# taldatech/soft-intro-vae-pytorch

Hardware: AMD Instinct MI355X
Metric: training images/sec (whole node) at 256x256 bs128 (higher is better)
Workload: dtype f32; 1 GPU; soft_intro_vae celeb256 256x256 zdim=512 channels=[64, 128, 256, 512, 512, 512], full E-step + D-step iteration; global_batch=128, per_gpu_batch=128, parallelism=dp1, decoder_forward_reuse=True, hip_graph=False, batchnorm=local

## Files before the change

### soft-intro-vae-pytorch_amd/csrc/bn_fused.hip

```cpp
#include "bn_fused_common.h"
#include <stdlib.h>

namespace {

struct BnFusedArgs {
  const float* dy;
  const float* y;
  const float* x;
  const unsigned char* mask;
  const float* mean;
  const float* invstd;
  const float* gamma;
  const float* beta;
  float* dx;
  float* dz;
  float* dgamma;
  float* dbeta;
  double* part;
  double* sums;
  unsigned* bar;
  double count;
  float slope;
  int C, H, W, Bs, nseg;
  int l2_qpp, l2_qw;
  int spc, cpg, ngroups, nx;
  int nsub;
  int local;
  int dzmode;
  int pf;
  unsigned spin_limit;
#ifdef BF_TIMING
  unsigned long long* ts;
#endif
};
#ifdef BF_TIMING
#define BF_STAMP(K) \
  if (t == 0 && a.ts) a.ts[((size_t)blockIdx.x * a.ngroups + grp) * 8 + (K)] = __builtin_amdgcn_s_memrealtime();
#else
#define BF_STAMP(K)
#endif

__device__ __forceinline__ void bf_sign_nibble(float4& g, unsigned nib, float slope) {
  g.x = (nib & 1u) ? g.x : g.x * slope;
  g.y = (nib & 2u) ? g.y : g.y * slope;
  g.z = (nib & 4u) ? g.z : g.z * slope;
  g.w = (nib & 8u) ? g.w : g.w * slope;
}
__device__ __forceinline__ void bf_sign_val(float4& g, const float4 v, float slope) {
  g.x = v.x > 0.f ? g.x : g.x * slope;
  g.y = v.y > 0.f ? g.y : g.y * slope;
  g.z = v.z > 0.f ? g.z : g.z * slope;
  g.w = v.w > 0.f ? g.w : g.w * slope;
}
__device__ __forceinline__ void bf_store4(__amdgpu_buffer_rsrc_t r, const float4 v, unsigned voff, unsigned soff) {
  typedef unsigned int u32x4_t __attribute__((ext_vector_type(4)));
  f32x4 f;
  f[0] = v.x;
  f[1] = v.y;
  f[2] = v.z;
  f[3] = v.w;
  __builtin_amdgcn_raw_buffer_store_b128(__builtin_bit_cast(u32x4_t, f), r, (int)voff, (int)soff, 0);
}
#define BF_KEEP(V) asm volatile("" ::"v"((V).x), "v"((V).y), "v"((V).z), "v"((V).w));

template <int ACT, bool POOL, int NQ>
__global__ void __launch_bounds__(256, 2) bn_bwd_fused_kernel(BnFusedArgs a) {
  __shared__ double red[8];
  extern __shared__ __attribute__((aligned(16))) float4 bf_pfx[];
  const int t = threadIdx.x;
  const int wave64 = __builtin_amdgcn_readfirstlane(t >> 6) * 64;
  const bool pf = NQ <= 8 && a.pf != 0;
  constexpr int PFQ = NQ < 6 ? NQ : 6;
  const bool local = a.local != 0;
  const int nb_sub = local ? (int)gridDim.x : (int)gridDim.x / a.nsub;
  const int sub = (!local && (int)blockIdx.x >= nb_sub) ? 1 : 0;
  const int bid = (int)blockIdx.x - sub * nb_sub;
  unsigned* bar = a.bar + sub * BF_BAR_UINTS;
  unsigned* chcnt = a.bar + 2 * BF_BAR_UINTS;
  const int xcd = bid % a.nx;
  const unsigned bpx = (unsigned)(nb_sub / a.nx);
  __shared__ int bar_failed;
  unsigned target = 0, nbar = 0;
  if (t == 0 && !local) target = bf_load_u32(bar + (9 + xcd) * 32);
  const int C = a.C, W = a.W, HW = a.H * a.W;
  const int VC = a.nseg * C;
  const int nq = a.Bs << a.l2_qpp;
  const unsigned qpp_m = (1u << a.l2_qpp) - 1u, qw_m = (1u << a.l2_qw) - 1u;
  const int ci = local ? 0 : bid / a.spc, slab = local ? 0 : bid - ci * a.spc;
  const float slope = a.slope;
  const unsigned img_pitch = (unsigned)C * (unsigned)HW * 4u;
  const unsigned row_b = (unsigned)W * 4u;
  const unsigned long long win = ((unsigned long long)(a.Bs - 1) * C + 1ull) * HW * 4ull;

  float4 g0[NQ], g1[NQ], x0[NQ], x1[NQ];
#pragma unroll
  for (int j = 0; j < NQ; ++j) g0[j] = g1[j] = x0[j] = x1[j] = make_float4(0.f, 0.f, 0.f, 0.f);
  const unsigned qbase = (unsigned)(slab * (256 * NQ) + t);
  auto quad_off = [&](unsigned q) -> unsigned {
    const unsigned b = q >> a.l2_qpp, r = q & qpp_m, h2 = r >> a.l2_qw, w4 = r & qw_m;
    const unsigned off = b * img_pitch + (2u * h2 * (unsigned)W + 4u * w4) * 4u;
    return q < (unsigned)nq ? off : BF_OOB;
  };
  auto half_off = [&](unsigned q) -> unsigned {
    const unsigned b = q >> a.l2_qpp, r = q & qpp_m, h2 = r >> a.l2_qw, w4 = r & qw_m;
    const unsigned off = b * (img_pitch >> 2) + (h2 * (unsigned)(W >> 1) + 2u * w4) * 4u;
    return q < (unsigned)nq ? off : BF_OOB;
  };
  auto request_x = [&](int vcn) {
    const int segn = vcn / C, cn = vcn - segn * C;
    const __amdgpu_buffer_rsrc_t rxn = make_rsrc(a.x + ((size_t)segn * a.Bs * C + cn) * (size_t)HW, win);
#pragma unroll
    for (int j = 0; j < PFQ; ++j) {
      const unsigned vo = quad_off(qbase + j * 256);
      __builtin_amdgcn_raw_ptr_buffer_load_lds(rxn, (float __attribute__((address_space(3)))*)(bf_pfx + (2 * j) * 256 + wave64),
                                               16, (int)vo, 0, 0, 0);
      __builtin_amdgcn_raw_ptr_buffer_load_lds(rxn, (float __attribute__((address_space(3)))*)(bf_pfx + (2 * j + 1) * 256 + wave64),
                                               16, (int)vo, (int)row_b, 0, 0);
    }
  };
  if (pf && !local && ci < a.cpg && sub * a.cpg + ci < VC && sub < a.ngroups) request_x(sub * a.cpg + ci);
  for (int grp = sub; grp < (local ? 1 : a.ngroups); grp += a.nsub) {
    const int vc = local ? bid : grp * a.cpg + ci;
    const bool active = local ? true : (ci < a.cpg && vc < VC);
    double t1 = 0.0, t2 = 0.0;
    float m = 0.f, is = 0.f, gs = 0.f;
    int c = 0;
    size_t base = 0;
    BF_STAMP(0)
    if (active) {
      const int seg = vc / C;
      c = vc - seg * C;
      m = a.mean[vc];
      is = a.invstd[vc];
      gs = a.gamma[c] * is;
      const float bt = ACT == 2 ? a.beta[c] : 0.f;
      base = ((size_t)seg * a.Bs * C + c) * (size_t)HW;
      const __amdgpu_buffer_rsrc_t rx = make_rsrc(a.x + base, win);
      const __amdgpu_buffer_rsrc_t rdy = POOL ? make_rsrc(a.dy + (base >> 2), win >> 2) : make_rsrc(a.dy + base, win);
      unsigned nib[ACT == 3 ? NQ : 1];
#pragma unroll
      for (int j = 0; j < NQ; ++j) {
        const unsigned vo = quad_off(qbase + j * 256);
        BF_KEEP(x0[j]) BF_KEEP(x1[j]) BF_KEEP(g0[j]) BF_KEEP(g1[j])
        if (!pf || j >= PFQ) {
          x0[j] = buf_load_f32x4(rx, vo, 0);
          x1[j] = buf_load_f32x4(rx, vo, row_b);
        }
        if (POOL) {
          const float2 d = buf_load_f32x2(rdy, half_off(qbase + j * 256), 0);
          g0[j] = make_float4(0.25f * d.x, 0.25f * d.x, 0.25f * d.y, 0.25f * d.y);
          g1[j] = g0[j];
        } else {
          g0[j] = buf_load_f32x4(rdy, vo, 0);
          g1[j] = buf_load_f32x4(rdy, vo, row_b);
        }
        if (ACT == 3) {
          const __amdgpu_buffer_rsrc_t rm = make_rsrc(a.mask + (base >> 3), win >> 5);
          const unsigned mo = vo == BF_OOB ? BF_OOB : (vo >> 5);
          const unsigned b0_ = (unsigned)__builtin_amdgcn_raw_buffer_load_b8(rm, (int)mo, 0, 0);
          const unsigned b1_ = (unsigned)__builtin_amdgcn_raw_buffer_load_b8(rm, (int)mo, (int)(W >> 3), 0);
          nib[j] = b0_ | (b1_ << 8);
        }
        if (ACT == 1) {
          const __amdgpu_buffer_rsrc_t ry = make_rsrc(a.y + base, win);
          bf_sign_val(g0[j], buf_load_f32x4(ry, vo, 0), slope);
          bf_sign_val(g1[j], buf_load_f32x4(ry, vo, row_b), slope);
        }
      }
      if (pf) {
#pragma unroll
        for (int j = 0; j < PFQ; ++j) {
          x0[j] = bf_pfx[(2 * j) * 256 + t];
          x1[j] = bf_pfx[(2 * j + 1) * 256 + t];
        }
      }
      double s1 = 0.0, s2 = 0.0;
#ifdef BF_TIMING
      asm volatile("s_waitcnt vmcnt(0)" ::: "memory");
#endif
      BF_STAMP(1)
#pragma unroll
      for (int j = 0; j < NQ; ++j) {
        if (ACT == 3) {
          const unsigned sh = (quad_off(qbase + j * 256) >> 4) & 1u ? 4u : 0u;
          bf_sign_nibble(g0[j], (nib[j] >> sh) & 0xfu, slope);
          bf_sign_nibble(g1[j], (nib[j] >> (8u + sh)) & 0xfu, slope);
        }
        if (ACT == 2) {
          float4 v = make_float4((x0[j].x - m) * gs + bt, (x0[j].y - m) * gs + bt, (x0[j].z - m) * gs + bt,
                                 (x0[j].w - m) * gs + bt);
          bf_sign_val(g0[j], v, slope);
          v = make_float4((x1[j].x - m) * gs + bt, (x1[j].y - m) * gs + bt, (x1[j].z - m) * gs + bt,
                          (x1[j].w - m) * gs + bt);
          bf_sign_val(g1[j], v, slope);
        }
        x0[j] = make_float4((x0[j].x - m) * is, (x0[j].y - m) * is, (x0[j].z - m) * is, (x0[j].w - m) * is);
        x1[j] = make_float4((x1[j].x - m) * is, (x1[j].y - m) * is, (x1[j].z - m) * is, (x1[j].w - m) * is);
        const float q1 = ((g0[j].x + g0[j].y) + (g0[j].z + g0[j].w)) + ((g1[j].x + g1[j].y) + (g1[j].z + g1[j].w));
        const float q2 = ((g0[j].x * x0[j].x + g0[j].y * x0[j].y) + (g0[j].z * x0[j].z + g0[j].w * x0[j].w)) +
                         ((g1[j].x * x1[j].x + g1[j].y * x1[j].y) + (g1[j].z * x1[j].z + g1[j].w * x1[j].w));
        s1 += (double)q1;
        s2 += (double)q2;
      }
      block_sum2<256>(s1, s2, red);
      if (local) {
        t1 = s1;
        t2 = s2;
      } else if (t == 0) {
        __hip_atomic_store(a.part + ((size_t)vc * a.spc + slab) * 2 + 0, s1, __ATOMIC_RELAXED, __HIP_MEMORY_SCOPE_AGENT);
        __hip_atomic_store(a.part + ((size_t)vc * a.spc + slab) * 2 + 1, s2, __ATOMIC_RELAXED, __HIP_MEMORY_SCOPE_AGENT);
      }
    }
    BF_STAMP(2)
    if (!local) {
      if (t == 0) {
        ++target;
        bf_grid_arrive(bar, xcd, a.nx, bpx, nbar++);
      }
      BF_STAMP(3)
      if (pf) {
        const int vcn = (grp + a.nsub) * a.cpg + ci;
        if (grp + a.nsub < a.ngroups && ci < a.cpg && vcn < VC) request_x(vcn);
      }
      if (t == 0) bar_failed = bf_grid_wait(bar, a.bar + BF_POISON_WORD, xcd, target, a.spin_limit) ? 0 : 1;
      BF_STAMP(4)
      __syncthreads();
      if (bar_failed) return;
      if (!active) continue;
      for (int s = t; s < a.spc; s += 512) {
        const int sb = s + 256 < a.spc ? s + 256 : s;
        const double p1 = bf_load_f64(a.part + ((size_t)vc * a.spc + s) * 2 + 0);
        const double p2 = bf_load_f64(a.part + ((size_t)vc * a.spc + s) * 2 + 1);
        const double q1 = bf_load_f64(a.part + ((size_t)vc * a.spc + sb) * 2 + 0);
        const double q2 = bf_load_f64(a.part + ((size_t)vc * a.spc + sb) * 2 + 1);
        t1 += p1;
        t2 += p2;
        if (s + 256 < a.spc) {
          t1 += q1;
          t2 += q2;
        }
      }
      block_sum2<256>(t1, t2, red);
    }
    const float c1 = (float)(t1 / a.count), c2 = (float)(t2 / a.count);
    BF_STAMP(5)
    if (slab == 0 && t == 0 && (a.dgamma != nullptr || a.dbeta != nullptr)) {
      if (a.nseg == 1) {
        if (a.dbeta) a.dbeta[c] = (float)t1;
        if (a.dgamma) a.dgamma[c] = (float)t2;
      } else {
        __hip_atomic_store(a.sums + (size_t)vc * 2 + 0, t1, __ATOMIC_RELAXED, __HIP_MEMORY_SCOPE_AGENT);
        __hip_atomic_store(a.sums + (size_t)vc * 2 + 1, t2, __ATOMIC_RELAXED, __HIP_MEMORY_SCOPE_AGENT);
        asm volatile("s_waitcnt vmcnt(0)" ::: "memory");
        const unsigned done = __hip_atomic_fetch_add(chcnt + c, 1u, __ATOMIC_RELAXED, __HIP_MEMORY_SCOPE_AGENT);
        if (done == (unsigned)a.nseg - 1u) {
          double u1 = 0.0, u2 = 0.0;
          for (int g = 0; g < a.nseg; ++g) {
            u1 += bf_load_f64(a.sums + (size_t)(g * C + c) * 2 + 0);
            u2 += bf_load_f64(a.sums + (size_t)(g * C + c) * 2 + 1);
          }
          if (a.dbeta) a.dbeta[c] = (float)u1;
          if (a.dgamma) a.dgamma[c] = (float)u2;
          __hip_atomic_store(chcnt + c, 0u, __ATOMIC_RELAXED, __HIP_MEMORY_SCOPE_AGENT);
        }
      }
    }
    const __amdgpu_buffer_rsrc_t rdx = make_rsrc(a.dx + base, win);
    const __amdgpu_buffer_rsrc_t rdz = a.dzmode == 2 ? make_rsrc(a.dz + (base >> 2), win >> 2)
                                                     : make_rsrc(a.dzmode == 1 ? a.dz + base : a.dx + base, win);
#pragma unroll
    for (int j = 0; j < NQ; ++j) {
      const unsigned vo = quad_off(qbase + j * 256);
      x0[j].x = gs * (g0[j].x - c1 - x0[j].x * c2);
      x0[j].y = gs * (g0[j].y - c1 - x0[j].y * c2);
      x0[j].z = gs * (g0[j].z - c1 - x0[j].z * c2);
      x0[j].w = gs * (g0[j].w - c1 - x0[j].w * c2);
      x1[j].x = gs * (g1[j].x - c1 - x1[j].x * c2);
      x1[j].y = gs * (g1[j].y - c1 - x1[j].y * c2);
      x1[j].z = gs * (g1[j].z - c1 - x1[j].z * c2);
      x1[j].w = gs * (g1[j].w - c1 - x1[j].w * c2);
      if (vo == BF_OOB) continue;
      bf_store4(rdx, x0[j], vo, 0);
      bf_store4(rdx, x1[j], vo, row_b);
      if (a.dzmode == 1) {
        bf_store4(rdz, g0[j], vo, 0);
        bf_store4(rdz, g1[j], vo, row_b);
      } else if (a.dzmode == 2) {
        const float sa = (g0[j].x + g0[j].y) + (g1[j].x + g1[j].y);
        const float sb = (g0[j].z + g0[j].w) + (g1[j].z + g1[j].w);
        buf_store_f32x2(rdz, sa, sb, half_off(qbase + j * 256), 0);
      }
    }
    BF_STAMP(6)
#ifdef BF_TIMING
    asm volatile("s_waitcnt vmcnt(0)" ::: "memory");
    BF_STAMP(7)
#endif
  }
  if (t == 0 && bid == 0 && nbar != 0u) bf_grid_reset(bar, a.nx);
  asm volatile("s_waitcnt vmcnt(0)" ::: "memory");
#pragma unroll
  for (int j = 0; j < NQ; ++j) { BF_KEEP(x0[j]) BF_KEEP(x1[j]) BF_KEEP(g0[j]) BF_KEEP(g1[j]) }
}

struct BfPlan {
  int nq_per_thread;
  int spc, cpg, ngroups, nb_sub, nsub;
  int local;
};

static bool bf_occupancy_ok() {
  static int ok = -1;
  if (ok < 0) {
    int ndev = 0, n = 0;
    if (hipGetDeviceCount(&ndev) != hipSuccess || ndev <= 0) {
      (void)hipGetLastError();
      ok = 1;
    } else {
      hipError_t e = hipSuccess;
      int n8 = 0;
      if (e == hipSuccess) e = hipOccupancyMaxActiveBlocksPerMultiprocessor(&n8, bn_bwd_fused_kernel<3, false, 8>, 256, 48 * 1024);
      if (e == hipSuccess) e = hipOccupancyMaxActiveBlocksPerMultiprocessor(&n, bn_bwd_fused_kernel<3, false, 10>, 256, 0);
      if (e == hipSuccess && n8 < n) n = n8;
      ok = (e != hipSuccess || n >= 2) ? 1 : 0;
      if (e != hipSuccess) (void)hipGetLastError();
    }
  }
  return ok == 1;
}

static bool bf_plan(int Bs, int VC, int HW, int max_nq, BfPlan* out) {
  const long long nq = (long long)Bs * HW / 8;
  out->local = 0;
  for (int NQ : {4, 8, 10}) {
    if (NQ > max_nq || nq > 256LL * NQ) continue;
    out->nq_per_thread = NQ;
    out->spc = 1;
    out->cpg = 1;
    out->ngroups = VC;
    out->nb_sub = VC;
    out->nsub = 1;
    out->local = 1;
    return true;
  }
  if (!bf_persistent_allowed() || !bf_occupancy_ok()) return false;
  for (int nsub = 2; nsub >= 1; --nsub) {
    const int nb_sub = sivae_num_cus() * (nsub == 2 ? 1 : 2);
    double best = 0.0;
    bool found = false;
    static int force_nq = -1;
    if (force_nq < 0) {
      const char* e = getenv("SIVAE_BN_FUSED_NQ");
      force_nq = e ? atoi(e) : 0;
    }
    for (int NQ : {10, 8, 4}) {
      if (NQ > max_nq) continue;
      if (force_nq > 0 && NQ != force_nq && NQ <= max_nq && force_nq <= max_nq) continue;
      const long long slabq = 256LL * NQ;
      const long long spc = (nq + slabq - 1) / slabq;
      if (spc > nb_sub) continue;
      const int cpg = (int)(nb_sub / spc);
      const int ngroups = (VC + cpg - 1) / cpg;
      const double cost = (double)((ngroups + nsub - 1) / nsub) * (8.0 + 2.5 * NQ);
      if (!found || cost < best) {
        best = cost;
        found = true;
        out->nq_per_thread = NQ;
        out->spc = (int)spc;
        out->cpg = cpg;
        out->ngroups = ngroups;
        out->nb_sub = nb_sub;
        out->nsub = nsub;
      }
    }
    if (found) return true;
  }
  return false;
}

static inline bool is_pow2(int v) { return v > 0 && (v & (v - 1)) == 0; }

#ifdef BF_TIMING
static unsigned long long* bf_timing_buffer = nullptr;
#endif

}

#ifdef BF_TIMING
extern "C" void sivae_debug_bf_timing(unsigned long long* buf) { bf_timing_buffer = buf; }
extern "C" int sivae_debug_bf_plan(int B, int C, int H, int W, int seg_images, int max_nq, int* out6) {
  BfPlan p;
  if (!bf_plan(seg_images, (B / seg_images) * C, H * W, max_nq, &p)) return -1;
  out6[0] = p.nq_per_thread; out6[1] = p.spc; out6[2] = p.cpg; out6[3] = p.ngroups; out6[4] = p.nb_sub; out6[5] = p.nsub;
  return 0;
}
#endif

extern "C" int sivae_bn_bwd_fused_supported(int B, int C, int H, int W, int seg_images) {
  if (B <= 0 || C <= 0 || C > BF_CH_COUNTERS || !is_pow2(H) || !is_pow2(W) || H < 2 || W < 4) return 0;
  if (seg_images <= 0 || B % seg_images != 0) return 0;
  if ((long long)B * C * H * W >= 0xffffffffLL) return 0;
  if ((long long)seg_images * C * H * W * 4 >= 0xfffffe00LL) return 0;
  BfPlan p;
  return bf_plan(seg_images, (B / seg_images) * C, H * W, 8, &p) ? 1 : 0;
}

extern "C" int sivae_bn_bwd_fused_poison_word() { return BF_POISON_WORD; }

extern "C" size_t sivae_bn_bwd_fused_workspace_bytes(int B, int C, int H, int W, int seg_images) {
  if (!sivae_bn_bwd_fused_supported(B, C, H, W, seg_images)) return 0;
  const int VC = (B / seg_images) * C;
  BfPlan p;
  size_t worst = 0;
  for (int mq : {10, 8, 4})
    if (bf_plan(seg_images, VC, H * W, mq, &p) && (size_t)p.spc > worst) worst = (size_t)p.spc;
  return ((size_t)VC * worst * 2 + (size_t)VC * 2) * sizeof(double);
}

extern "C" int sivae_bn_bwd_fused_state_uints() { return 2 * BF_BAR_UINTS + BF_CH_COUNTERS; }

extern "C" int sivae_bn_bwd_fused(const float* dy, const float* y, const unsigned char* mask, const float* x,
                                  const float* mean, const float* invstd, const float* gamma, const float* beta,
                                  int act_mode, float slope, float* dx, float* dz_out, float* dgamma, float* dbeta, int B,
                                  int C, int H, int W, int dy_pooled, int dz_sum, int seg_images, unsigned int* state,
                                  void* workspace, size_t workspace_bytes, hipStream_t stream) {
  if (!dy || !x || !mean || !invstd || !gamma || !dx || !state) return SIVAE_ERR_NULL;
  if (act_mode < 0 || act_mode > 3) return SIVAE_ERR_MODE;
  if (act_mode == 1 && !y) return SIVAE_ERR_NULL;
  if (act_mode == 2 && !beta) return SIVAE_ERR_NULL;
  if (act_mode == 3 && !mask) return SIVAE_ERR_NULL;
  if (act_mode == 3 && (W & 7)) return SIVAE_ERR_SHAPE;
  if (dy_pooled && dz_sum) return SIVAE_ERR_MODE;
  if (dz_sum && !dz_out) return SIVAE_ERR_NULL;
  if (!sivae_bn_bwd_fused_supported(B, C, H, W, seg_images)) return SIVAE_ERR_SHAPE;
  if (((uintptr_t)dy & 15u) || ((uintptr_t)x & 15u) || ((uintptr_t)dx & 15u) || (dz_out && ((uintptr_t)dz_out & 15u)) ||
      (y && ((uintptr_t)y & 15u)))
    return SIVAE_ERR_SHAPE;
  const int nseg = B / seg_images, VC = nseg * C;
  BfPlan p;
  if (!bf_plan(seg_images, VC, H * W, act_mode == 1 ? 8 : 10, &p)) return SIVAE_ERR_SHAPE;
  const size_t need = ((size_t)VC * p.spc * 2 + (size_t)VC * 2) * sizeof(double);
  if (!workspace || workspace_bytes < need) return SIVAE_ERR_WORKSPACE;
  BnFusedArgs a;
  a.dy = dy;
  a.y = y;
  a.x = x;
  a.mask = mask;
  a.mean = mean;
  a.invstd = invstd;
  a.gamma = gamma;
  a.beta = beta;
  a.dx = dx;
  a.dz = dz_out;
  a.dgamma = dgamma;
  a.dbeta = dbeta;
  a.part = (double*)workspace;
  a.sums = a.part + (size_t)VC * p.spc * 2;
  a.bar = state;
  a.count = (double)seg_images * H * W;
  a.slope = slope;
  a.C = C;
  a.H = H;
  a.W = W;
  a.Bs = seg_images;
  a.nseg = nseg;
  a.l2_qpp = ilog2_exact(H * W / 8);
  a.l2_qw = ilog2_exact(W / 4);
  a.spc = p.spc;
  a.cpg = p.cpg;
  a.ngroups = p.ngroups;
  a.nx = (!p.local && p.nb_sub % 8 == 0) ? 8 : 1;
  a.nsub = p.nsub;
  a.local = p.local;
  a.dzmode = !dz_out ? 0 : (dz_sum ? 2 : 1);
  a.spin_limit = bf_spin_limit();
#ifdef BF_TIMING
  a.ts = bf_timing_buffer;
#endif
  static int pf_on = -1;
  if (pf_on < 0) {
    const char* e = getenv("SIVAE_BN_FUSED_PREFETCH");
    pf_on = (e && e[0] == '0') ? 0 : 1;
  }
  a.pf = (pf_on && !p.local && p.nq_per_thread <= 8 && p.ngroups > p.nsub) ? 1 : 0;
  const size_t lds = a.pf ? (size_t)(p.nq_per_thread < 6 ? p.nq_per_thread : 6) * 2 * 256 * sizeof(float4) : 0;
  const dim3 grid((unsigned)(p.local ? VC : p.nsub * p.nb_sub)), block(256);
#define BF_LAUNCH(A, P, Q) hipLaunchKernelGGL((bn_bwd_fused_kernel<A, P, Q>), grid, block, lds, stream, a);
#define BF_NQ(A, P)                                 \
  {                                                 \
    if (p.nq_per_thread == 10) BF_LAUNCH(A, P, 10) \
    else if (p.nq_per_thread == 8) BF_LAUNCH(A, P, 8) \
    else BF_LAUNCH(A, P, 4)                         \
  }
#define BF_ACT(A)              \
  {                            \
    if (dy_pooled) BF_NQ(A, true) else BF_NQ(A, false) \
  }
  if (act_mode == 0) BF_ACT(0) else if (act_mode == 1) BF_ACT(1) else if (act_mode == 2) BF_ACT(2) else BF_ACT(3)
#undef BF_ACT
#undef BF_NQ
#undef BF_LAUNCH
  return sivae_launch_status();
}
```

Before: 339.1 img/s.

## Keep pooled BN-backward gradients packed to allow larger per-thread quad counts

For the pooled-dy path without the y-based activation, the fused BN backward kernel now keeps the raw float2 pooled gradient and a packed sign mask per quad. It rebuilds the expanded float4 gradients on the fly in both the reduction and dx phases, instead of holding four float4 gradient registers per quad. The freed registers let the planner choose 12 or 16 quads per thread for this variant, and LDS prefetch is enabled for it. The aim is fewer slabs, fewer grid-barrier partial sums and better latency hiding. It adds recomputation, fixed fma ordering and a small rotating buffer with explicit vmcnt waits for dz stores, at the risk of register pressure lowering occupancy.

```diff
diff --git a/soft-intro-vae-pytorch_amd/csrc/bn_fused.hip b/soft-intro-vae-pytorch_amd/csrc/bn_fused.hip
--- a/soft-intro-vae-pytorch_amd/csrc/bn_fused.hip
+++ b/soft-intro-vae-pytorch_amd/csrc/bn_fused.hip
@@ -52,6 +52,25 @@
   g.z = v.z > 0.f ? g.z : g.z * slope;
   g.w = v.w > 0.f ? g.w : g.w * slope;
 }
+template <int ACT>
+__device__ __forceinline__ float4 bf_pooled_dz(const float2 d, unsigned nib, float slope) {
+  float4 g = make_float4(0.25f * d.x, 0.25f * d.x, 0.25f * d.y, 0.25f * d.y);
+  if (ACT != 0) bf_sign_nibble(g, nib, slope);
+  return g;
+}
+__device__ __forceinline__ float bf_dot8_fixed(const float4 h0, const float4 h1, const float4 x0, const float4 x1) {
+#pragma clang fp contract(off)
+  const float a = __builtin_fmaf(h0.y, x0.y, h0.x * x0.x), b = __builtin_fmaf(h0.w, x0.w, h0.z * x0.z);
+  const float c = __builtin_fmaf(h1.y, x1.y, h1.x * x1.x), d = __builtin_fmaf(h1.w, x1.w, h1.z * x1.z);
+  return (a + b) + (c + d);
+}
+__device__ __forceinline__ float bf_dx_fixed(float gs, float h, float c1, float xh, float c2) {
+#pragma clang fp contract(off)
+  return gs * __builtin_fmaf(-xh, c2, h - c1);
+}
+__device__ __forceinline__ unsigned bf_sign_bits(const float4 v) {
+  return (v.x > 0.f ? 1u : 0u) | (v.y > 0.f ? 2u : 0u) | (v.z > 0.f ? 4u : 0u) | (v.w > 0.f ? 8u : 0u);
+}
 __device__ __forceinline__ void bf_store4(__amdgpu_buffer_rsrc_t r, const float4 v, unsigned voff, unsigned soff) {
   typedef unsigned int u32x4_t __attribute__((ext_vector_type(4)));
   f32x4 f;
@@ -69,7 +88,8 @@
   extern __shared__ __attribute__((aligned(16))) float4 bf_pfx[];
   const int t = threadIdx.x;
   const int wave64 = __builtin_amdgcn_readfirstlane(t >> 6) * 64;
-  const bool pf = NQ <= 8 && a.pf != 0;
+  constexpr bool PK = POOL && ACT != 1;
+  const bool pf = (NQ <= 8 || PK) && a.pf != 0;
   constexpr int PFQ = NQ < 6 ? NQ : 6;
   const bool local = a.local != 0;
   const int nb_sub = local ? (int)gridDim.x : (int)gridDim.x / a.nsub;
@@ -92,10 +112,35 @@
   const unsigned row_b = (unsigned)W * 4u;
   const unsigned long long win = ((unsigned long long)(a.Bs - 1) * C + 1ull) * HW * 4ull;
 
-  float4 g0[NQ], g1[NQ], x0[NQ], x1[NQ];
-#pragma unroll
-  for (int j = 0; j < NQ; ++j) g0[j] = g1[j] = x0[j] = x1[j] = make_float4(0.f, 0.f, 0.f, 0.f);
+  constexpr int NG = PK ? 1 : NQ;
+  constexpr int NP = PK ? NQ : 1;
+  float4 g0[NG], g1[NG], x0[NQ], x1[NQ];
+  float2 dd[NP];
+  unsigned sg[NP];
+  constexpr int ZR = NQ >= 16 ? 2 : (NQ >= 4 ? 4 : NQ);
+  float4 z0[ZR], z1[ZR];
+#pragma unroll
+  for (int j = 0; j < NQ; ++j) x0[j] = x1[j] = make_float4(0.f, 0.f, 0.f, 0.f);
+#pragma unroll
+  for (int j = 0; j < NG; ++j) g0[j] = g1[j] = make_float4(0.f, 0.f, 0.f, 0.f);
+#pragma unroll
+  for (int j = 0; j < ZR; ++j) z0[j] = z1[j] = make_float4(0.f, 0.f, 0.f, 0.f);
+#pragma unroll
+  for (int j = 0; j < NP; ++j) {
+    dd[j] = make_float2(0.f, 0.f);
+    sg[j] = 0u;
+  }
+  auto row_nibbles = [&](unsigned s, unsigned vo, unsigned& n0, unsigned& n1) {
+    const unsigned sh = (ACT == 3 && ((vo >> 4) & 1u)) ? 4u : 0u;
+    n0 = (s >> sh) & 0xfu;
+    n1 = (s >> (8u + sh)) & 0xfu;
+  };
   const unsigned qbase = (unsigned)(slab * (256 * NQ) + t);
+  auto phase_base = [&]() -> unsigned {
+    unsigned q = qbase;
+    if constexpr (PK) asm volatile("" : "+v"(q));
+    return q;
+  };
   auto quad_off = [&](unsigned q) -> unsigned {
     const unsigned b = q >> a.l2_qpp, r = q & qpp_m, h2 = r >> a.l2_qw, w4 = r & qw_m;
     const unsigned off = b * img_pitch + (2u * h2 * (unsigned)W + 4u * w4) * 4u;
@@ -137,17 +182,21 @@
       base = ((size_t)seg * a.Bs * C + c) * (size_t)HW;
       const __amdgpu_buffer_rsrc_t rx = make_rsrc(a.x + base, win);
       const __amdgpu_buffer_rsrc_t rdy = POOL ? make_rsrc(a.dy + (base >> 2), win >> 2) : make_rsrc(a.dy + base, win);
-      unsigned nib[ACT == 3 ? NQ : 1];
+      unsigned nib[(ACT == 3 && !PK) ? NQ : 1];
+      const unsigned qb1 = phase_base();
 #pragma unroll
       for (int j = 0; j < NQ; ++j) {
-        const unsigned vo = quad_off(qbase + j * 256);
-        BF_KEEP(x0[j]) BF_KEEP(x1[j]) BF_KEEP(g0[j]) BF_KEEP(g1[j])
+        const unsigned vo = quad_off(qb1 + j * 256);
+        BF_KEEP(x0[j]) BF_KEEP(x1[j])
+        if constexpr (!PK) { BF_KEEP(g0[j]) BF_KEEP(g1[j]) }
         if (!pf || j >= PFQ) {
           x0[j] = buf_load_f32x4(rx, vo, 0);
           x1[j] = buf_load_f32x4(rx, vo, row_b);
         }
-        if (POOL) {
-          const float2 d = buf_load_f32x2(rdy, half_off(qbase + j * 256), 0);
+        if constexpr (PK) {
+          dd[j] = buf_load_f32x2(rdy, half_off(qb1 + j * 256), 0);
+        } else if (POOL) {
+          const float2 d = buf_load_f32x2(rdy, half_off(qb1 + j * 256), 0);
           g0[j] = make_float4(0.25f * d.x, 0.25f * d.x, 0.25f * d.y, 0.25f * d.y);
           g1[j] = g0[j];
         } else {
@@ -159,9 +208,10 @@
           const unsigned mo = vo == BF_OOB ? BF_OOB : (vo >> 5);
           const unsigned b0_ = (unsigned)__builtin_amdgcn_raw_buffer_load_b8(rm, (int)mo, 0, 0);
           const unsigned b1_ = (unsigned)__builtin_amdgcn_raw_buffer_load_b8(rm, (int)mo, (int)(W >> 3), 0);
-          nib[j] = b0_ | (b1_ << 8);
-        }
-        if (ACT == 1) {
+          if constexpr (PK) sg[j] = b0_ | (b1_ << 8);
+          else nib[j] = b0_ | (b1_ << 8);
+        }
+        if constexpr (ACT == 1) {
           const __amdgpu_buffer_rsrc_t ry = make_rsrc(a.y + base, win);
           bf_sign_val(g0[j], buf_load_f32x4(ry, vo, 0), slope);
           bf_sign_val(g1[j], buf_load_f32x4(ry, vo, row_b), slope);
@@ -181,24 +231,47 @@
       BF_STAMP(1)
 #pragma unroll
       for (int j = 0; j < NQ; ++j) {
-        if (ACT == 3) {
-          const unsigned sh = (quad_off(qbase + j * 256) >> 4) & 1u ? 4u : 0u;
-          bf_sign_nibble(g0[j], (nib[j] >> sh) & 0xfu, slope);
-          bf_sign_nibble(g1[j], (nib[j] >> (8u + sh)) & 0xfu, slope);
-        }
-        if (ACT == 2) {
-          float4 v = make_float4((x0[j].x - m) * gs + bt, (x0[j].y - m) * gs + bt, (x0[j].z - m) * gs + bt,
-                                 (x0[j].w - m) * gs + bt);
-          bf_sign_val(g0[j], v, slope);
-          v = make_float4((x1[j].x - m) * gs + bt, (x1[j].y - m) * gs + bt, (x1[j].z - m) * gs + bt,
-                          (x1[j].w - m) * gs + bt);
-          bf_sign_val(g1[j], v, slope);
-        }
-        x0[j] = make_float4((x0[j].x - m) * is, (x0[j].y - m) * is, (x0[j].z - m) * is, (x0[j].w - m) * is);
-        x1[j] = make_float4((x1[j].x - m) * is, (x1[j].y - m) * is, (x1[j].z - m) * is, (x1[j].w - m) * is);
-        const float q1 = ((g0[j].x + g0[j].y) + (g0[j].z + g0[j].w)) + ((g1[j].x + g1[j].y) + (g1[j].z + g1[j].w));
-        const float q2 = ((g0[j].x * x0[j].x + g0[j].y * x0[j].y) + (g0[j].z * x0[j].z + g0[j].w * x0[j].w)) +
-                         ((g1[j].x * x1[j].x + g1[j].y * x1[j].y) + (g1[j].z * x1[j].z + g1[j].w * x1[j].w));
+        float4 h0, h1;
+        if constexpr (PK) {
+          unsigned n0 = 0u, n1 = 0u;
+          if (ACT == 3) row_nibbles(sg[j], quad_off(qb1 + j * 256), n0, n1);
+          if (ACT == 2) {
+            n0 = bf_sign_bits(make_float4((x0[j].x - m) * gs + bt, (x0[j].y - m) * gs + bt, (x0[j].z - m) * gs + bt,
+                                          (x0[j].w - m) * gs + bt));
+            n1 = bf_sign_bits(make_float4((x1[j].x - m) * gs + bt, (x1[j].y - m) * gs + bt, (x1[j].z - m) * gs + bt,
+                                          (x1[j].w - m) * gs + bt));
+            sg[j] = n0 | (n1 << 8);
+          }
+          x0[j] = make_float4((x0[j].x - m) * is, (x0[j].y - m) * is, (x0[j].z - m) * is, (x0[j].w - m) * is);
+          x1[j] = make_float4((x1[j].x - m) * is, (x1[j].y - m) * is, (x1[j].z - m) * is, (x1[j].w - m) * is);
+          h0 = bf_pooled_dz<ACT>(dd[j], n0, slope);
+          h1 = bf_pooled_dz<ACT>(dd[j], n1, slope);
+        } else {
+          if (ACT == 3) {
+            const unsigned sh = (quad_off(qb1 + j * 256) >> 4) & 1u ? 4u : 0u;
+            bf_sign_nibble(g0[j], (nib[j] >> sh) & 0xfu, slope);
+            bf_sign_nibble(g1[j], (nib[j] >> (8u + sh)) & 0xfu, slope);
+          }
+          if (ACT == 2) {
+            float4 v = make_float4((x0[j].x - m) * gs + bt, (x0[j].y - m) * gs + bt, (x0[j].z - m) * gs + bt,
+                                   (x0[j].w - m) * gs + bt);
+            bf_sign_val(g0[j], v, slope);
+            v = make_float4((x1[j].x - m) * gs + bt, (x1[j].y - m) * gs + bt, (x1[j].z - m) * gs + bt,
+                            (x1[j].w - m) * gs + bt);
+            bf_sign_val(g1[j], v, slope);
+          }
+          x0[j] = make_float4((x0[j].x - m) * is, (x0[j].y - m) * is, (x0[j].z - m) * is, (x0[j].w - m) * is);
+          x1[j] = make_float4((x1[j].x - m) * is, (x1[j].y - m) * is, (x1[j].z - m) * is, (x1[j].w - m) * is);
+          h0 = g0[j];
+          h1 = g1[j];
+        }
+        const float q1 = ((h0.x + h0.y) + (h0.z + h0.w)) + ((h1.x + h1.y) + (h1.z + h1.w));
+        float q2;
+        if constexpr (POOL)
+          q2 = bf_dot8_fixed(h0, h1, x0[j], x1[j]);
+        else
+          q2 = ((h0.x * x0[j].x + h0.y * x0[j].y) + (h0.z * x0[j].z + h0.w * x0[j].w)) +
+               ((h1.x * x1[j].x + h1.y * x1[j].y) + (h1.z * x1[j].z + h1.w * x1[j].w));
         s1 += (double)q1;
         s2 += (double)q2;
       }
@@ -265,30 +338,68 @@
         }
       }
     }
+    const unsigned qb2 = phase_base();
     const __amdgpu_buffer_rsrc_t rdx = make_rsrc(a.dx + base, win);
     const __amdgpu_buffer_rsrc_t rdz = a.dzmode == 2 ? make_rsrc(a.dz + (base >> 2), win >> 2)
                                                      : make_rsrc(a.dzmode == 1 ? a.dz + base : a.dx + base, win);
 #pragma unroll
     for (int j = 0; j < NQ; ++j) {
-      const unsigned vo = quad_off(qbase + j * 256);
-      x0[j].x = gs * (g0[j].x - c1 - x0[j].x * c2);
-      x0[j].y = gs * (g0[j].y - c1 - x0[j].y * c2);
-      x0[j].z = gs * (g0[j].z - c1 - x0[j].z * c2);
-      x0[j].w = gs * (g0[j].w - c1 - x0[j].w * c2);
-      x1[j].x = gs * (g1[j].x - c1 - x1[j].x * c2);
-      x1[j].y = gs * (g1[j].y - c1 - x1[j].y * c2);
-      x1[j].z = gs * (g1[j].z - c1 - x1[j].z * c2);
-      x1[j].w = gs * (g1[j].w - c1 - x1[j].w * c2);
+      const unsigned vo = quad_off(qb2 + j * 256);
+      float4 h0, h1;
+      if constexpr (PK) {
+        unsigned n0 = 0u, n1 = 0u;
+        if (ACT != 0) row_nibbles(sg[j], vo, n0, n1);
+        h0 = bf_pooled_dz<ACT>(dd[j], n0, slope);
+        h1 = bf_pooled_dz<ACT>(dd[j], n1, slope);
+      } else {
+        h0 = g0[j];
+        h1 = g1[j];
+      }
+      if constexpr (POOL) {
+        x0[j].x = bf_dx_fixed(gs, h0.x, c1, x0[j].x, c2);
+        x0[j].y = bf_dx_fixed(gs, h0.y, c1, x0[j].y, c2);
+        x0[j].z = bf_dx_fixed(gs, h0.z, c1, x0[j].z, c2);
+        x0[j].w = bf_dx_fixed(gs, h0.w, c1, x0[j].w, c2);
+        x1[j].x = bf_dx_fixed(gs, h1.x, c1, x1[j].x, c2);
+        x1[j].y = bf_dx_fixed(gs, h1.y, c1, x1[j].y, c2);
+        x1[j].z = bf_dx_fixed(gs, h1.z, c1, x1[j].z, c2);
+        x1[j].w = bf_dx_fixed(gs, h1.w, c1, x1[j].w, c2);
+      } else {
+        x0[j].x = gs * (h0.x - c1 - x0[j].x * c2);
+        x0[j].y = gs * (h0.y - c1 - x0[j].y * c2);
+        x0[j].z = gs * (h0.z - c1 - x0[j].z * c2);
+        x0[j].w = gs * (h0.w - c1 - x0[j].w * c2);
+        x1[j].x = gs * (h1.x - c1 - x1[j].x * c2);
+        x1[j].y = gs * (h1.y - c1 - x1[j].y * c2);
+        x1[j].z = gs * (h1.z - c1 - x1[j].z * c2);
+        x1[j].w = gs * (h1.w - c1 - x1[j].w * c2);
+      }
       if (vo == BF_OOB) continue;
-      bf_store4(rdx, x0[j], vo, 0);
-      bf_store4(rdx, x1[j], vo, row_b);
-      if (a.dzmode == 1) {
-        bf_store4(rdz, g0[j], vo, 0);
-        bf_store4(rdz, g1[j], vo, row_b);
-      } else if (a.dzmode == 2) {
-        const float sa = (g0[j].x + g0[j].y) + (g1[j].x + g1[j].y);
-        const float sb = (g0[j].z + g0[j].w) + (g1[j].z + g1[j].w);
-        buf_store_f32x2(rdz, sa, sb, half_off(qbase + j * 256), 0);
+      if constexpr (PK) {
+        if (a.dzmode == 1) {
+          if (j == 0) asm volatile("s_waitcnt vmcnt(0)" ::: "memory");
+          else if (j >= ZR) asm volatile("s_waitcnt vmcnt(%0)" ::"n"(4 * (ZR - 1)) : "memory");
+          BF_KEEP(z0[j % ZR]) BF_KEEP(z1[j % ZR])
+          z0[j % ZR] = h0;
+          z1[j % ZR] = h1;
+        }
+        bf_store4(rdx, x0[j], vo, 0);
+        bf_store4(rdx, x1[j], vo, row_b);
+        if (a.dzmode == 1) {
+          bf_store4(rdz, z0[j % ZR], vo, 0);
+          bf_store4(rdz, z1[j % ZR], vo, row_b);
+        }
+      } else {
+        bf_store4(rdx, x0[j], vo, 0);
+        bf_store4(rdx, x1[j], vo, row_b);
+        if (a.dzmode == 1) {
+          bf_store4(rdz, g0[j], vo, 0);
+          bf_store4(rdz, g1[j], vo, row_b);
+        } else if (a.dzmode == 2) {
+          const float sa = (g0[j].x + g0[j].y) + (g1[j].x + g1[j].y);
+          const float sb = (g0[j].z + g0[j].w) + (g1[j].z + g1[j].w);
+          buf_store_f32x2(rdz, sa, sb, half_off(qb2 + j * 256), 0);
+        }
       }
     }
     BF_STAMP(6)
@@ -300,8 +411,19 @@
   if (t == 0 && bid == 0 && nbar != 0u) bf_grid_reset(bar, a.nx);
   asm volatile("s_waitcnt vmcnt(0)" ::: "memory");
 #pragma unroll
-  for (int j = 0; j < NQ; ++j) { BF_KEEP(x0[j]) BF_KEEP(x1[j]) BF_KEEP(g0[j]) BF_KEEP(g1[j]) }
-}
+  for (int j = 0; j < NQ; ++j) {
+    BF_KEEP(x0[j]) BF_KEEP(x1[j])
+    if constexpr (!PK) { BF_KEEP(g0[j]) BF_KEEP(g1[j]) }
+  }
+  if constexpr (PK) {
+    if (a.dzmode == 1) {
+#pragma unroll
+      for (int j = 0; j < ZR; ++j) { BF_KEEP(z0[j]) BF_KEEP(z1[j]) }
+    }
+  }
+}
+
+constexpr int BF_PACKED_MAX_NQ = 16;
 
 struct BfPlan {
   int nq_per_thread;
@@ -318,10 +440,12 @@
       ok = 1;
     } else {
       hipError_t e = hipSuccess;
-      int n8 = 0;
+      int n8 = 0, n16 = 0;
       if (e == hipSuccess) e = hipOccupancyMaxActiveBlocksPerMultiprocessor(&n8, bn_bwd_fused_kernel<3, false, 8>, 256, 48 * 1024);
       if (e == hipSuccess) e = hipOccupancyMaxActiveBlocksPerMultiprocessor(&n, bn_bwd_fused_kernel<3, false, 10>, 256, 0);
+      if (e == hipSuccess) e = hipOccupancyMaxActiveBlocksPerMultiprocessor(&n16, bn_bwd_fused_kernel<3, true, 16>, 256, 48 * 1024);
       if (e == hipSuccess && n8 < n) n = n8;
+      if (e == hipSuccess && n16 < n) n = n16;
       ok = (e != hipSuccess || n >= 2) ? 1 : 0;
       if (e != hipSuccess) (void)hipGetLastError();
     }
@@ -332,7 +456,13 @@
 static bool bf_plan(int Bs, int VC, int HW, int max_nq, BfPlan* out) {
   const long long nq = (long long)Bs * HW / 8;
   out->local = 0;
-  for (int NQ : {4, 8, 10}) {
+  static int force_nq = -1;
+  if (force_nq < 0) {
+    const char* e = getenv("SIVAE_BN_FUSED_NQ");
+    force_nq = e ? atoi(e) : 0;
+  }
+  if (force_nq > 0 && force_nq <= 10 && max_nq > 10) max_nq = 10;
+  for (int NQ : {4, 8, 10, 12, 16}) {
     if (NQ > max_nq || nq > 256LL * NQ) continue;
     out->nq_per_thread = NQ;
     out->spc = 1;
@@ -348,12 +478,7 @@
     const int nb_sub = sivae_num_cus() * (nsub == 2 ? 1 : 2);
     double best = 0.0;
     bool found = false;
-    static int force_nq = -1;
-    if (force_nq < 0) {
-      const char* e = getenv("SIVAE_BN_FUSED_NQ");
-      force_nq = e ? atoi(e) : 0;
-    }
-    for (int NQ : {10, 8, 4}) {
+    for (int NQ : {16, 12, 10, 8, 4}) {
       if (NQ > max_nq) continue;
       if (force_nq > 0 && NQ != force_nq && NQ <= max_nq && force_nq <= max_nq) continue;
       const long long slabq = 256LL * NQ;
@@ -412,7 +537,7 @@
   const int VC = (B / seg_images) * C;
   BfPlan p;
   size_t worst = 0;
-  for (int mq : {10, 8, 4})
+  for (int mq : {16, 12, 10, 8, 4})
     if (bf_plan(seg_images, VC, H * W, mq, &p) && (size_t)p.spc > worst) worst = (size_t)p.spc;
   return ((size_t)VC * worst * 2 + (size_t)VC * 2) * sizeof(double);
 }
@@ -438,7 +563,8 @@
     return SIVAE_ERR_SHAPE;
   const int nseg = B / seg_images, VC = nseg * C;
   BfPlan p;
-  if (!bf_plan(seg_images, VC, H * W, act_mode == 1 ? 8 : 10, &p)) return SIVAE_ERR_SHAPE;
+  const bool packed = dy_pooled && act_mode != 1;
+  if (!bf_plan(seg_images, VC, H * W, act_mode == 1 ? 8 : (packed ? BF_PACKED_MAX_NQ : 10), &p)) return SIVAE_ERR_SHAPE;
   const size_t need = ((size_t)VC * p.spc * 2 + (size_t)VC * 2) * sizeof(double);
   if (!workspace || workspace_bytes < need) return SIVAE_ERR_WORKSPACE;
   BnFusedArgs a;
@@ -482,7 +608,7 @@
     const char* e = getenv("SIVAE_BN_FUSED_PREFETCH");
     pf_on = (e && e[0] == '0') ? 0 : 1;
   }
-  a.pf = (pf_on && !p.local && p.nq_per_thread <= 8 && p.ngroups > p.nsub) ? 1 : 0;
+  a.pf = (pf_on && !p.local && (p.nq_per_thread <= 8 || packed) && p.ngroups > p.nsub) ? 1 : 0;
   const size_t lds = a.pf ? (size_t)(p.nq_per_thread < 6 ? p.nq_per_thread : 6) * 2 * 256 * sizeof(float4) : 0;
   const dim3 grid((unsigned)(p.local ? VC : p.nsub * p.nb_sub)), block(256);
 #define BF_LAUNCH(A, P, Q) hipLaunchKernelGGL((bn_bwd_fused_kernel<A, P, Q>), grid, block, lds, stream, a);
@@ -492,12 +618,21 @@
     else if (p.nq_per_thread == 8) BF_LAUNCH(A, P, 8) \
     else BF_LAUNCH(A, P, 4)                         \
   }
+#define BF_NQ_PACKED(A)                                 \
+  {                                                     \
+    if (p.nq_per_thread == 16) BF_LAUNCH(A, true, 16)   \
+    else if (p.nq_per_thread == 12) BF_LAUNCH(A, true, 12) \
+    else BF_NQ(A, true)                                 \
+  }
 #define BF_ACT(A)              \
   {                            \
-    if (dy_pooled) BF_NQ(A, true) else BF_NQ(A, false) \
-  }
-  if (act_mode == 0) BF_ACT(0) else if (act_mode == 1) BF_ACT(1) else if (act_mode == 2) BF_ACT(2) else BF_ACT(3)
+    if (dy_pooled) BF_NQ_PACKED(A) else BF_NQ(A, false) \
+  }
+  if (act_mode == 0) BF_ACT(0) else if (act_mode == 1) {
+    if (dy_pooled) BF_NQ(1, true) else BF_NQ(1, false)
+  } else if (act_mode == 2) BF_ACT(2) else BF_ACT(3)
 #undef BF_ACT
+#undef BF_NQ_PACKED
 #undef BF_NQ
 #undef BF_LAUNCH
   return sivae_launch_status();
```

Result: no change. 340.0 img/s, median of 6 (+0.3%).
